# i2Nav-WHU/IC-GVINS

Measured on AMD Instinct MI355X. Metric: frames/s at 1280x720, 300 feats, 10-KF window; residual/Jacobian eval/s, higher is better.
Workload: dtype u8/int64 front-end (f32/f64 solves), f64 factors

## Files before the change

### ic-gvins_amd/csrc/image.hip

```cpp
#include <algorithm>

#include "icg_internal.h"

#define PRE_MAX_JOBS 64
struct pre_jobs {
    const uint8_t *src[PRE_MAX_JOBS];
    int32_t slot[PRE_MAX_JOBS];
    int stride;
    const int32_t *slot_ind;
};
__device__ __forceinline__ int pre_job_slot(const pre_jobs &j, int b) { return j.slot_ind ? j.slot_ind[b] : j.slot[b]; }

__global__ void k_bgr2gray(const uint8_t *bgr, int w, int h, int sstride, size_t sbatch, uint8_t *gray, int gstride,
                           size_t gbatch) {
    int x = blockIdx.x * blockDim.x + threadIdx.x;
    int y = blockIdx.y;
    int b = blockIdx.z;
    if (x >= w) return;
    const uint8_t *p = bgr + (size_t) b * sbatch + (size_t) y * sstride + 3 * x;
    gray[(size_t) b * gbatch + (size_t) y * gstride + x] =
        (uint8_t) ((p[0] * 1868 + p[1] * 9617 + p[2] * 4899 + 8192) >> 14);
}

__global__ void k_hist256(pre_jobs jobs, int w, int h, unsigned int *hist ) {
    __shared__ unsigned int sh[256];
    int b = blockIdx.y;
    sh[threadIdx.x] = 0;
    __syncthreads();
    const uint8_t *src = jobs.src[b];
    const int stride   = jobs.stride;
    int total          = src ? w * h : 0;
    for (int i = blockIdx.x * blockDim.x + threadIdx.x; i < total; i += gridDim.x * blockDim.x) {
        int y = i / w, x = i - y * w;
        atomicAdd(&sh[src[(size_t) y * stride + x]], 1u);
    }
    __syncthreads();
    if (sh[threadIdx.x]) atomicAdd(&hist[(size_t) b * 256 + threadIdx.x], sh[threadIdx.x]);
}

struct clahe_geom {
    int w, h, tw, th, clip;
    float lut_scale, inv_tw, inv_th;
};

__device__ __forceinline__ int wave_sum_i32(int v) {
    v += __builtin_amdgcn_update_dpp(0, v, 0xB1, 0xF, 0xF, false);
    v += __builtin_amdgcn_update_dpp(0, v, 0x4E, 0xF, 0xF, false);
    v += __builtin_amdgcn_update_dpp(0, v, 0x141, 0xF, 0xF, false);
    v += __builtin_amdgcn_update_dpp(0, v, 0x140, 0xF, 0xF, false);
    v += __builtin_amdgcn_update_dpp(0, v, 0x142, 0xA, 0xF, false);
    v += __builtin_amdgcn_update_dpp(0, v, 0x143, 0xC, 0xF, false);
    return __builtin_amdgcn_readlane(v, 63);
}
__device__ __forceinline__ int wave_scan_i32(int v) {
    v += __builtin_amdgcn_update_dpp(0, v, 0x111, 0xF, 0xF, true);
    v += __builtin_amdgcn_update_dpp(0, v, 0x112, 0xF, 0xF, true);
    v += __builtin_amdgcn_update_dpp(0, v, 0x114, 0xF, 0xF, true);
    v += __builtin_amdgcn_update_dpp(0, v, 0x118, 0xF, 0xF, true);
    v += __builtin_amdgcn_update_dpp(0, v, 0x142, 0xA, 0xF, false);
    v += __builtin_amdgcn_update_dpp(0, v, 0x143, 0xC, 0xF, false);
    return v;
}

__global__ __launch_bounds__(64) void k_clahe_lut(pre_jobs jobs, clahe_geom g, uint8_t *lut , int n_items) {
    __shared__ __attribute__((aligned(16))) unsigned int hist[256];
    const int lane = threadIdx.x;
    const int item = icg_xcd_chunked(blockIdx.x, n_items);
    if (item >= n_items) return;
    const int b    = item / (ICG_CLAHE_TILES * ICG_CLAHE_TILES);
    const int tile = item - b * (ICG_CLAHE_TILES * ICG_CLAHE_TILES);
    const int ty = tile / ICG_CLAHE_TILES, tx = tile - ty * ICG_CLAHE_TILES;
    const uint8_t *src = jobs.src[b];
    if (!src) return;
    const int stride   = jobs.stride;
    reinterpret_cast<uint4 *>(hist)[lane] = make_uint4(0, 0, 0, 0);
    __syncthreads();

    const int x_begin = tx * g.tw, x_end = x_begin + g.tw, y_begin = ty * g.th;
    const int xa  = x_begin & ~3;
    const int ndw = (((x_end + 3) & ~3) - xa) >> 2;
    const bool pad_small = g.th * ICG_CLAHE_TILES < 2 * g.h - 1;
    auto load_row_dword = [&](int r, int x) -> unsigned int {
        const uint8_t *row = src + (size_t) (pad_small ? icg_reflect1(y_begin + r, g.h) : icg_reflect101(y_begin + r, g.h)) * stride;
        if (x + 3 < g.w) return *reinterpret_cast<const unsigned int *>(row + x);
        unsigned int v = 0;
#pragma unroll
        for (int j = 0; j < 4; j++) v |= (unsigned int) row[icg_reflect101(x + j, g.w)] << (8 * j);
        return v;
    };
    const int nin = ndw - 2;
    const bool fast = nin >= 1 && nin <= 16 && y_begin + g.th <= g.h && xa + 4 * ndw <= g.w;
    if (fast) {
        const int d = lane & 15, q = lane >> 4;
        const bool on = d < nin;
        const uint8_t *p = src + (size_t) (y_begin + q) * stride + (xa + 4 * (on ? d + 1 : 1));
        unsigned char *hb = reinterpret_cast<unsigned char *>(hist);
        const size_t step = 4 * (size_t) stride;
        for (int r = q; r < g.th; r += 16, p += 4 * step) {
            unsigned int v[4];
            bool ok[4];
#pragma unroll
            for (int k = 0; k < 4; k++) {
                ok[k] = on && r + 4 * k < g.th;
                v[k]  = r + 4 * k < g.th ? *reinterpret_cast<const unsigned int *>(p + k * step) : 0u;
            }
#pragma unroll
            for (int k = 0; k < 4; k++) {
                if (ok[k]) {
                    atomicAdd(reinterpret_cast<unsigned int *>(hb + ((v[k] << 2) & 0x3fcu)), 1u);
                    atomicAdd(reinterpret_cast<unsigned int *>(hb + ((v[k] >> 6) & 0x3fcu)), 1u);
                    atomicAdd(reinterpret_cast<unsigned int *>(hb + ((v[k] >> 14) & 0x3fcu)), 1u);
                    atomicAdd(reinterpret_cast<unsigned int *>(hb + ((v[k] >> 22) & 0x3fcu)), 1u);
                }
            }
        }
    } else {
        {
            const int items = g.th * (nin > 0 ? nin : 0);
            const unsigned int magic = nin > 0 ? ((1u << 20) + (unsigned int) nin - 1u) / (unsigned int) nin : 0u;
            constexpr int CH = 9;
            for (int base = 0; base < items; base += 64 * CH) {
                unsigned int v[CH];
                bool ok[CH];
    #pragma unroll
                for (int k = 0; k < CH; k++) {
                    const int i = base + k * 64 + lane;
                    ok[k]       = i < items;
                    v[k]        = 0;
                    if (ok[k]) {
                        const int r = (int) (((unsigned int) i * magic) >> 20), d = 1 + i - r * nin;
                        v[k]        = load_row_dword(r, xa + 4 * d);
                    }
                }
    #pragma unroll
                for (int k = 0; k < CH; k++) {
                    if (ok[k]) {
    #pragma unroll
                        for (int j = 0; j < 4; j++) atomicAdd(&hist[(v[k] >> (8 * j)) & 0xff], 1u);
                    }
                }
            }
        }
    }
    {
        const int nedge = ndw >= 2 ? 2 : 1, items = g.th * nedge;
        for (int i = lane; i < items; i += 64) {
            const int r = nedge == 2 ? (i >> 1) : i, d = (nedge == 2 && (i & 1)) ? ndw - 1 : 0;
            const int x = xa + 4 * d;
            const unsigned int v = load_row_dword(r, x);
#pragma unroll
            for (int j = 0; j < 4; j++) {
                const int xx = x + j;
                if (xx >= x_begin && xx < x_end) atomicAdd(&hist[(v >> (8 * j)) & 0xff], 1u);
            }
        }
    }
    __syncthreads();

    const uint4 h4 = reinterpret_cast<const uint4 *>(hist)[lane];
    int hv[4]      = {(int) h4.x, (int) h4.y, (int) h4.z, (int) h4.w};
    int excess     = 0;
#pragma unroll
    for (int j = 0; j < 4; j++) {
        if (hv[j] > g.clip) {
            excess += hv[j] - g.clip;
            hv[j] = g.clip;
        }
    }
    const int clipped   = wave_sum_i32(excess);
    const int batch_add = clipped / 256;
    const int residual  = clipped - batch_add * 256;
    int step            = residual ? 256 / residual : 1;
    if (step < 1) step = 1;
    int run = 0;
#pragma unroll
    for (int j = 0; j < 4; j++) {
        const int t = 4 * lane + j;
        hv[j] += batch_add;
        if (residual != 0 && (t % step) == 0 && (t / step) < residual) hv[j]++;
        run += hv[j];
        hv[j] = run;
    }
    const int incl = wave_scan_i32(run);
    const int excl = incl - run;
    unsigned int packed = 0;
#pragma unroll
    for (int j = 0; j < 4; j++) {
        const float f = rintf((float) (excl + hv[j]) * g.lut_scale);
        int iv        = (int) f;
        iv            = iv < 0 ? 0 : (iv > 255 ? 255 : iv);
        packed |= (unsigned int) iv << (8 * j);
    }
    reinterpret_cast<unsigned int *>(lut + ((size_t) b * ICG_CLAHE_TILES * ICG_CLAHE_TILES + tile) * 256)[lane] = packed;
}

#define CLAHE_CHUNK 256
#define CLAHE_MAXCOLS 24
#define CLAHE_FCOLS 8

typedef float f32x2 __attribute__((ext_vector_type(2)));

template <bool FLT>
__device__ __forceinline__ void clahe_apply_body(const pre_jobs &jobs, const clahe_geom &g, const uint8_t *lut, uint8_t *frames, size_t slot_bytes,
                                                 int dpitch, unsigned int *slut, int strip, int chunk, int b, int t, int dslot, int p_lo, int npairs,
                                                 int x_begin) {
    const int T = ICG_CLAHE_TILES;
    int ty1 = strip - 1, ty2 = strip;
    if (ty1 < 0) ty1 = 0;
    if (ty2 > T - 1) ty2 = T - 1;
    const unsigned int *blut = reinterpret_cast<const unsigned int *>(lut + (size_t) b * T * T * 256);
    for (int i = t; i < npairs * 64; i += 256) {
        const int p = p_lo + (i >> 6), v4 = i & 63;
        int c1 = p - 1, c2 = p;
        if (c1 < 0) c1 = 0;
        if (c2 > T - 1) c2 = T - 1;
        const unsigned int A = blut[(ty1 * T + c1) * 64 + v4], B = blut[(ty1 * T + c2) * 64 + v4];
        const unsigned int C = blut[(ty2 * T + c1) * 64 + v4], D = blut[(ty2 * T + c2) * 64 + v4];
        if (FLT) {
            float4 *dst = reinterpret_cast<float4 *>(slut) + 4 * i;
#define CL_F(w, k) ((float) (((w) >> (8 * (k))) & 0xffu))
            dst[0] = make_float4(CL_F(A, 0), CL_F(B, 0), CL_F(C, 0), CL_F(D, 0));
            dst[1] = make_float4(CL_F(A, 1), CL_F(B, 1), CL_F(C, 1), CL_F(D, 1));
            dst[2] = make_float4(CL_F(A, 2), CL_F(B, 2), CL_F(C, 2), CL_F(D, 2));
            dst[3] = make_float4(CL_F(A, 3), CL_F(B, 3), CL_F(C, 3), CL_F(D, 3));
#undef CL_F
        } else {
            const unsigned int ab01 = __builtin_amdgcn_perm(B, A, 0x05010400u), ab23 = __builtin_amdgcn_perm(B, A, 0x07030602u);
            const unsigned int cd01 = __builtin_amdgcn_perm(D, C, 0x05010400u), cd23 = __builtin_amdgcn_perm(D, C, 0x07030602u);
            uint4 e;
            e.x = __builtin_amdgcn_perm(cd01, ab01, 0x05040100u);
            e.y = __builtin_amdgcn_perm(cd01, ab01, 0x07060302u);
            e.z = __builtin_amdgcn_perm(cd23, ab23, 0x05040100u);
            e.w = __builtin_amdgcn_perm(cd23, ab23, 0x07060302u);
            reinterpret_cast<uint4 *>(slut)[i] = e;
        }
    }
    __syncthreads();

    const int wave = t >> 6, lane = t & 63;
    const int x0 = x_begin + lane * 4;
    int pofs[4];
    float xa[4], xa1[4];
#pragma unroll
    for (int k = 0; k < 4; k++) {
        const int x     = x0 + k;
        const float txf = x * g.inv_tw - 0.5f;
        const int tx1   = (int) floorf(txf);
        xa[k]           = txf - tx1;
        xa1[k]          = 1.0f - xa[k];
        int p           = tx1 + 1 - p_lo;
        p               = p < 0 ? 0 : (p > npairs - 1 ? npairs - 1 : p);
        pofs[k]         = p << 8;
    }
    if (x0 >= g.w) return;

    int y_lo = (strip - 1) * g.th + g.th / 2 - 2;
    int y_hi = strip * g.th + g.th / 2 + 3;
    if (y_lo < 0) y_lo = 0;
    if (y_hi > g.h) y_hi = g.h;
    const uint8_t *src = jobs.src[b];
    const int stride   = jobs.stride;
    uint8_t *dst       = frames + (size_t) dslot * slot_bytes;
    if (FLT) {
        const float4 *sf = reinterpret_cast<const float4 *>(slut);
        for (int y = y_lo + wave; y < y_hi; y += 4) {
            const float tyf = y * g.inv_th - 0.5f;
            const int tyr   = (int) floorf(tyf);
            if (tyr != strip - 1) continue;
            const float ya = tyf - tyr, ya1 = 1.0f - ya;
            const unsigned int pin = *reinterpret_cast<const unsigned int *>(src + (size_t) y * stride + x0);
            const float4 e0 = sf[pofs[0] + (pin & 0xff)], e1 = sf[pofs[1] + ((pin >> 8) & 0xff)];
            const float4 e2 = sf[pofs[2] + ((pin >> 16) & 0xff)], e3 = sf[pofs[3] + (pin >> 24)];
            const float r0 = (e0.x * xa1[0] + e0.y * xa[0]) * ya1 + (e0.z * xa1[0] + e0.w * xa[0]) * ya;
            const float r1 = (e1.x * xa1[1] + e1.y * xa[1]) * ya1 + (e1.z * xa1[1] + e1.w * xa[1]) * ya;
            const float r2 = (e2.x * xa1[2] + e2.y * xa[2]) * ya1 + (e2.z * xa1[2] + e2.w * xa[2]) * ya;
            const float r3 = (e3.x * xa1[3] + e3.y * xa[3]) * ya1 + (e3.z * xa1[3] + e3.w * xa[3]) * ya;
            const unsigned int m0 = __float_as_uint(r0 + 12582912.f), m1 = __float_as_uint(r1 + 12582912.f);
            const unsigned int m2 = __float_as_uint(r2 + 12582912.f), m3 = __float_as_uint(r3 + 12582912.f);
            const unsigned int lo = __builtin_amdgcn_perm(m1, m0, 0x0c0c0400u), hi = __builtin_amdgcn_perm(m3, m2, 0x0c0c0400u);
            *reinterpret_cast<unsigned int *>(dst + (size_t) y * dpitch + x0) = __builtin_amdgcn_perm(hi, lo, 0x05040100u);
        }
        return;
    }
    const f32x2 XA01 = {xa[0], xa[1]}, XA23 = {xa[2], xa[3]}, XB01 = {xa1[0], xa1[1]}, XB23 = {xa1[2], xa1[3]};
    for (int y = y_lo + wave; y < y_hi; y += 4) {
        const float tyf = y * g.inv_th - 0.5f;
        const int tyr   = (int) floorf(tyf);
        if (tyr != strip - 1) continue;
        const float ya = tyf - tyr, ya1 = 1.0f - ya;
        const unsigned int pin = *reinterpret_cast<const unsigned int *>(src + (size_t) y * stride + x0);
        const unsigned int e0 = slut[pofs[0] + (pin & 0xff)], e1 = slut[pofs[1] + ((pin >> 8) & 0xff)];
        const unsigned int e2 = slut[pofs[2] + ((pin >> 16) & 0xff)], e3 = slut[pofs[3] + (pin >> 24)];
#define CL_B(e, k) ((float) (((e) >> (8 * (k))) & 0xffu))
        const f32x2 A01 = {CL_B(e0, 0), CL_B(e1, 0)}, B01 = {CL_B(e0, 1), CL_B(e1, 1)};
        const f32x2 C01 = {CL_B(e0, 2), CL_B(e1, 2)}, D01 = {CL_B(e0, 3), CL_B(e1, 3)};
        const f32x2 A23 = {CL_B(e2, 0), CL_B(e3, 0)}, B23 = {CL_B(e2, 1), CL_B(e3, 1)};
        const f32x2 C23 = {CL_B(e2, 2), CL_B(e3, 2)}, D23 = {CL_B(e2, 3), CL_B(e3, 3)};
#undef CL_B
        const f32x2 r01 = (A01 * XB01 + B01 * XA01) * ya1 + (C01 * XB01 + D01 * XA01) * ya;
        const f32x2 r23 = (A23 * XB23 + B23 * XA23) * ya1 + (C23 * XB23 + D23 * XA23) * ya;
        const float res[4] = {r01.x, r01.y, r23.x, r23.y};
        unsigned int pout = 0;
#pragma unroll
        for (int k = 0; k < 4; k++) {
            const int iv = (int) rintf(res[k]);
            pout |= (unsigned int) (iv < 0 ? 0 : (iv > 255 ? 255 : iv)) << (8 * k);
        }
        *reinterpret_cast<unsigned int *>(dst + (size_t) y * dpitch + x0) = pout;
    }
}

__global__ __launch_bounds__(256) void k_clahe_apply(pre_jobs jobs, clahe_geom g, const uint8_t *lut, uint8_t *frames,
                                                     size_t slot_bytes, int dpitch) {
    __shared__ __attribute__((aligned(16))) unsigned int slut[CLAHE_FCOLS * 256 * 4];
    static_assert(CLAHE_FCOLS * 4 >= CLAHE_MAXCOLS, "the byte form must fit the same array");
    const int strip = blockIdx.x;
    const int chunk = blockIdx.y;
    const int b     = blockIdx.z;
    const int t     = threadIdx.x;
    const int dslot = pre_job_slot(jobs, b);
    if (!jobs.src[b] || dslot < 0) return;
    const int x_begin = chunk * CLAHE_CHUNK;
    int x_end         = x_begin + CLAHE_CHUNK;
    if (x_end > g.w) x_end = g.w;
    const int p_lo   = (int) floorf(x_begin * g.inv_tw - 0.5f) + 1;
    const int p_hi   = (int) floorf((x_end - 1) * g.inv_tw - 0.5f) + 1;
    const int npairs = p_hi - p_lo + 1;
    if (npairs <= CLAHE_FCOLS)
        clahe_apply_body<true>(jobs, g, lut, frames, slot_bytes, dpitch, slut, strip, chunk, b, t, dslot, p_lo, npairs, x_begin);
    else
        clahe_apply_body<false>(jobs, g, lut, frames, slot_bytes, dpitch, slut, strip, chunk, b, t, dslot, p_lo, npairs, x_begin);
}

#define PR_STRIP_OUT 128
struct pr_sel {
    unsigned int a, b, t, v;
};
typedef unsigned int pr_u3 __attribute__((ext_vector_type(3)));
__device__ __forceinline__ pr_u3 pr_load(const uint8_t *row, unsigned int wx) {
    typedef pr_u3 __attribute__((aligned(4))) u3a;
    return *reinterpret_cast<const u3a *>(row + wx);
}
template <bool EDGE> __device__ __forceinline__ unsigned int pr_hsum(const pr_u3 E, const pr_sel &S) {
    unsigned int A, B, V4;
    if (EDGE) {
        A  = __builtin_amdgcn_perm(E.y, E.x, S.a);
        B  = __builtin_amdgcn_perm(E.y, E.x, S.b);
        V4 = __builtin_amdgcn_perm(E.z, __builtin_amdgcn_perm(E.y, E.x, S.t), S.v);
    } else {
        A  = __builtin_amdgcn_alignbyte(E.y, E.x, 2);
        B  = E.y;
        V4 = E.z & 0xffu;
    }
    const unsigned int h0 = __builtin_amdgcn_udot4(B, 0x00010000u, __builtin_amdgcn_udot4(A, 0x04060401u, 0u, false), false);
    const unsigned int h1 = __builtin_amdgcn_udot4(B, 0x04060401u, V4, false);
    return h0 | (h1 << 16);
}

template <bool EDGE>
__device__ __forceinline__ void pr_band(const uint8_t *src, int sh, int spitch, uint8_t *dst, int dpitch, int i0, int i1, unsigned int wx,
                                        const pr_sel &S, unsigned int dcol, bool store) {
    auto srow = [&](int r) { return src + (unsigned int) __builtin_amdgcn_readfirstlane(icg_reflect1(r, sh) * spitch); };
    unsigned int hA = pr_hsum<EDGE>(pr_load(srow(2 * i0 - 2), wx), S), hB = pr_hsum<EDGE>(pr_load(srow(2 * i0 - 1), wx), S);
    unsigned int hC = pr_hsum<EDGE>(pr_load(srow(2 * i0), wx), S);
// ... 38 lines not shown
        S.t = 0x0c0c0c00u | (unsigned int) (ix[6] & 7);
        S.v = ix[6] >= 8 ? (0x0c0c0c04u + (unsigned int) (ix[6] - 8)) : 0x0c0c0c00u;
    }
    const int i0 = band * band_rows, i1 = min(i0 + band_rows, dh);
    if (i0 >= i1) return;
    const uint8_t *src = slot + src_off;
    uint8_t *dst       = slot + dst_off;
    const bool store   = oj < dw;
    if (edge)
        pr_band<true>(src, sh, spitch, dst, dpitch, i0, i1, (unsigned int) wx, S, (unsigned int) oj, store);
    else
        pr_band<false>(src, sh, spitch, dst, dpitch, i0, i1, (unsigned int) wx, S, (unsigned int) oj, store);
}

__global__ void k_hist_mean(int n, const unsigned int *hist, int w, int h, double *mean) {
    const int k = blockIdx.x * blockDim.x + threadIdx.x;
    if (k >= n) return;
    double acc = 0;
    for (int i = 0; i < 256; i++) {
        const float hf = (float) hist[(size_t) k * 256 + i];
        acc += hf * (float) i / 256.0;
    }
    mean[k] = acc / ((double) w * h);
}

static int preprocess_impl(icg_ctx *ctx, int n, const int32_t *slots, const int32_t *d_slot_ind, const uint8_t *const *images, int stride, int channels,
                           int src_on_device, double *hist_mean, double *d_hist_mean) {
    if (!ctx || n < 0 || (n > 0 && ((!slots && !d_slot_ind) || !images))) return ICG_ERR_INVALID;
    if (n == 0) return ICG_OK;
    if (n > ctx->cfg.max_batch) return icg_fail(ctx, ICG_ERR_CAPACITY, "preprocess batch %d > max_batch %d", n, ctx->cfg.max_batch);
    if (channels != 1 && channels != 3) return icg_fail(ctx, ICG_ERR_INVALID, "channels must be 1 or 3");
    const int w = ctx->cfg.width, h = ctx->cfg.height;
    if (stride < w * channels) return icg_fail(ctx, ICG_ERR_INVALID, "stride too small");
    for (int k = 0; k < n && slots; k++)
        if (slots[k] < 0 || slots[k] >= ctx->cfg.n_slots || !images[k]) return icg_fail(ctx, ICG_ERR_INVALID, "bad slot/image %d", k);
    ICG_HIP(ctx, hipSetDevice(ctx->cfg.device));
    const bool want_hist = hist_mean || d_hist_mean;

    const int T = ICG_CLAHE_TILES;
    int ew = w, eh = h;
    if (w % T != 0 || h % T != 0) {
        ew = w + (T - w % T);
        eh = h + (T - h % T);
    }
    clahe_geom g;
    g.w = w;
    g.h = h;
    g.tw = ew / T;
    g.th = eh / T;
    int area    = g.tw * g.th;
    g.lut_scale = 255.0f / area;
    g.clip      = (int) (3.0 * area / 256);
    if (g.clip < 1) g.clip = 1;
    g.inv_tw = 1.0f / g.tw;
    g.inv_th = 1.0f / g.th;
    static_assert(ICG_CLAHE_TILES + 1 <= CLAHE_MAXCOLS, "k_clahe_apply's staged LUT must hold every interpolation column pair");

    const size_t raw_batch = (size_t) ctx->raw_pitch * h;
    hipMemcpyKind kind     = src_on_device ? hipMemcpyDeviceToDevice : hipMemcpyHostToDevice;
    unsigned int *d_hist   = nullptr;
    if (want_hist) {
        if (int rcd = icg_arena_drain(ctx)) return rcd;
        ctx->arena_off = 0;
        int rc         = icg_arena_reserve(ctx, sizeof(unsigned int) * 256 * (size_t) n + 4096);
        if (rc) return rc;
        d_hist = icg_d<unsigned int>(ctx, icg_arena_alloc(ctx, sizeof(unsigned int) * 256 * (size_t) n));
// ... 23 lines not shown
            bool direct = src_on_device && (stride % 4 == 0);
            for (int k = 0; k < m && direct; k++) direct = (((uintptr_t) images[base + k]) % 4) == 0;
            if (direct) {
                for (int k = 0; k < m; k++) jobs.src[k] = images[base + k];
                jobs.stride = stride;
            } else {
                const bool linear = stride == w && ctx->raw_pitch == w;
                for (int k = 0; k < m; k++) {
                    uint8_t *dst = ctx->d_raw + (size_t) (base + k) * raw_batch;
                    if (!images[base + k]) {
                        jobs.src[k] = nullptr;
                        continue;
                    }
                    if (linear)
                        ICG_HIP(ctx, hipMemcpyAsync(dst, images[base + k], (size_t) w * h, kind, ctx->stream));
                    else
                        ICG_HIP(ctx, hipMemcpy2DAsync(dst, ctx->raw_pitch, images[base + k], stride, w, h, kind, ctx->stream));
                    jobs.src[k] = dst;
                }
                jobs.stride = ctx->raw_pitch;
            }
        }
        if (want_hist) {
            icg_prof_scope ps(ctx, "hist256");
            hipLaunchKernelGGL(k_hist256, dim3(64, m), dim3(256), 0, ctx->stream, jobs, w, h, d_hist + (size_t) base * 256);
        }
        uint8_t *lut = ctx->d_lut + (size_t) base * T * T * 256;
        {
            icg_prof_scope ps(ctx, "clahe_lut");
            hipLaunchKernelGGL(k_clahe_lut, dim3(icg_xcd_grid(T * T * m)), dim3(64), 0, ctx->stream, jobs, g, lut, T * T * m);
        }
        {
            icg_prof_scope ps(ctx, "clahe_apply");
            hipLaunchKernelGGL(k_clahe_apply, dim3(T + 1, (w + CLAHE_CHUNK - 1) / CLAHE_CHUNK, m), dim3(256), 0, ctx->stream, jobs,
                               g, lut, ctx->d_frames, ctx->slot_bytes, ctx->lv[0].pitch);
        }
        for (int l = 1; l < ctx->n_levels; l++) {
            icg_prof_scope ps(ctx, "pyrdown_rows");
            const icg_level &a = ctx->lv[l - 1], &bb = ctx->lv[l];
            const int n_strips = (bb.w + PR_STRIP_OUT - 1) / PR_STRIP_OUT;
            const int band_rows = bb.h >= 256 ? 32 : bb.h >= 128 ? 16 : 8;
            const int n_bands   = (bb.h + band_rows - 1) / band_rows;
            const int n_tasks   = n_strips * n_bands * m;
            hipLaunchKernelGGL(k_pyrdown_rows, dim3(icg_xcd_grid(n_tasks)), dim3(64), 0, ctx->stream, ctx->d_frames, ctx->slot_bytes, jobs,
                               (unsigned int) a.off, a.w, a.h, a.pitch, (unsigned int) bb.off, bb.w, bb.h, bb.pitch, n_strips, n_bands, band_rows,
                               n_tasks);
        }
    }
    if (d_hist_mean) hipLaunchKernelGGL(k_hist_mean, dim3((n + 63) / 64), dim3(64), 0, ctx->stream, n, d_hist, w, h, d_hist_mean);
    ICG_HIP(ctx, hipGetLastError());
    if (d_hist_mean) ctx->arena_off = 0;
    if (!hist_mean) return ICG_OK;

    std::vector<unsigned int> hc((size_t) n * 256);
    ICG_HIP(ctx, hipMemcpyAsync(hc.data(), d_hist, sizeof(unsigned int) * 256 * (size_t) n, hipMemcpyDeviceToHost, ctx->stream));
    ICG_HIP(ctx, hipStreamSynchronize(ctx->stream));
    icg_prof_collect(ctx);
    for (int k = 0; k < n; k++) {
        double acc = 0;
        for (int i = 0; i < 256; i++) {
            float hf = (float) hc[(size_t) k * 256 + i];
            acc += hf * (float) i / 256.0;
        }
        hist_mean[k] = acc / ((double) w * h);
    }
    ctx->arena_off = 0;
    return ICG_OK;
// ... 24 lines not shown
```

Baseline: 162,800.

## Unify CLAHE histogram into templated row sweep and restructure LUT apply loop

Replaces the fast/slow/edge histogram paths in the CLAHE LUT kernel with a single templated sweep. Edge dwords are masked by redirecting out-of-tile bytes to per-lane dummy bins, and 24-bit unsigned row offsets replace size_t arithmetic. The clip-redistribution step uses a constant step table and shared-memory flags instead of per-bin divisions and modulos. The float interpolation apply loop ballots the active rows once per 64-row chunk, so waves no longer test each row individually. It also raises PRE_MAX_JOBS and adds a size check on the source plane so the 32-bit offsets stay valid.

```diff
diff --git a/ic-gvins_amd/csrc/image.hip b/ic-gvins_amd/csrc/image.hip
--- a/ic-gvins_amd/csrc/image.hip
+++ b/ic-gvins_amd/csrc/image.hip
@@ -2,7 +2,9 @@
 
 #include "icg_internal.h"
 
-#define PRE_MAX_JOBS 64
+#ifndef PRE_MAX_JOBS
+#define PRE_MAX_JOBS 192
+#endif
 struct pre_jobs {
     const uint8_t *src[PRE_MAX_JOBS];
     int32_t slot[PRE_MAX_JOBS];
@@ -62,8 +64,59 @@
     return v;
 }
 
+struct clahe_step_table {
+    int v[256];
+    constexpr clahe_step_table() : v() {
+        v[0] = 1;
+        for (int r = 1; r < 256; r++) v[r] = 256 / r;
+    }
+};
+__constant__ clahe_step_table c_clahe_step = clahe_step_table();
+
+template <int U, bool BYTES, bool BOTTOM, bool CHECK>
+__device__ __forceinline__ void clahe_hist_rows(const uint8_t *src, unsigned char *hb, const unsigned int (&am)[4], const unsigned int (&ov)[4],
+                                                const unsigned int (&xo)[4], int y0, int rs, int y_end, int h, unsigned int stride) {
+    unsigned int v[U];
+    bool ok[U];
+    const unsigned int ro0 = BOTTOM ? 0u : __umul24((unsigned int) y0, stride), rstep = (unsigned int) rs * stride;
+#pragma unroll
+    for (int k = 0; k < U; k++) {
+        const int y = y0 + k * rs;
+        ok[k] = !CHECK || y < y_end;
+        v[k]  = 0;
+        if (ok[k]) {
+            const unsigned int ro = BOTTOM ? __umul24((unsigned int) icg_reflect1(y, h), stride) : ro0 + (unsigned int) k * rstep;
+            if (BYTES) {
+                v[k] = (unsigned int) src[ro + xo[0]] | ((unsigned int) src[ro + xo[1]] << 8) | ((unsigned int) src[ro + xo[2]] << 16) |
+                       ((unsigned int) src[ro + xo[3]] << 24);
+            } else {
+                v[k] = *reinterpret_cast<const unsigned int *>(src + (ro + xo[0]));
+            }
+        }
+    }
+#pragma unroll
+    for (int k = 0; k < U; k++) {
+        if (ok[k]) {
+            atomicAdd(reinterpret_cast<unsigned int *>(hb + (((v[k] << 2) & am[0]) | ov[0])), 1u);
+            atomicAdd(reinterpret_cast<unsigned int *>(hb + (((v[k] >> 6) & am[1]) | ov[1])), 1u);
+            atomicAdd(reinterpret_cast<unsigned int *>(hb + (((v[k] >> 14) & am[2]) | ov[2])), 1u);
+            atomicAdd(reinterpret_cast<unsigned int *>(hb + (((v[k] >> 22) & am[3]) | ov[3])), 1u);
+        }
+    }
+}
+
+template <bool BYTES, bool BOTTOM>
+__device__ __forceinline__ void clahe_hist_sweep(const uint8_t *src, unsigned char *hb, const unsigned int (&am)[4], const unsigned int (&ov)[4],
+                                                 const unsigned int (&xo)[4], int y_begin, int q, int lgrs, int th, int h, unsigned int stride) {
+    const int rs = 1 << lgrs, full = th >> lgrs, y_end = y_begin + th;
+    int s = 0;
+    for (; s + 4 <= full; s += 4) clahe_hist_rows<4, BYTES, BOTTOM, false>(src, hb, am, ov, xo, y_begin + q + s * rs, rs, y_end, h, stride);
+    for (; s < full; s++) clahe_hist_rows<1, BYTES, BOTTOM, false>(src, hb, am, ov, xo, y_begin + q + s * rs, rs, y_end, h, stride);
+    if (th & (rs - 1)) clahe_hist_rows<1, BYTES, BOTTOM, true>(src, hb, am, ov, xo, y_begin + q + s * rs, rs, y_end, h, stride);
+}
+
 __global__ __launch_bounds__(64) void k_clahe_lut(pre_jobs jobs, clahe_geom g, uint8_t *lut , int n_items) {
-    __shared__ __attribute__((aligned(16))) unsigned int hist[256];
+    __shared__ __attribute__((aligned(16))) unsigned int hist[256 + 64];
     const int lane = threadIdx.x;
     const int item = icg_xcd_chunked(blockIdx.x, n_items);
     if (item >= n_items) return;
@@ -72,88 +125,40 @@
     const int ty = tile / ICG_CLAHE_TILES, tx = tile - ty * ICG_CLAHE_TILES;
     const uint8_t *src = jobs.src[b];
     if (!src) return;
-    const int stride   = jobs.stride;
+    const unsigned int stride = (unsigned int) jobs.stride;
     reinterpret_cast<uint4 *>(hist)[lane] = make_uint4(0, 0, 0, 0);
     __syncthreads();
 
     const int x_begin = tx * g.tw, x_end = x_begin + g.tw, y_begin = ty * g.th;
     const int xa  = x_begin & ~3;
     const int ndw = (((x_end + 3) & ~3) - xa) >> 2;
-    const bool pad_small = g.th * ICG_CLAHE_TILES < 2 * g.h - 1;
-    auto load_row_dword = [&](int r, int x) -> unsigned int {
-        const uint8_t *row = src + (size_t) (pad_small ? icg_reflect1(y_begin + r, g.h) : icg_reflect101(y_begin + r, g.h)) * stride;
-        if (x + 3 < g.w) return *reinterpret_cast<const unsigned int *>(row + x);
-        unsigned int v = 0;
-#pragma unroll
-        for (int j = 0; j < 4; j++) v |= (unsigned int) row[icg_reflect101(x + j, g.w)] << (8 * j);
-        return v;
-    };
-    const int nin = ndw - 2;
-    const bool fast = nin >= 1 && nin <= 16 && y_begin + g.th <= g.h && xa + 4 * ndw <= g.w;
-    if (fast) {
-        const int d = lane & 15, q = lane >> 4;
-        const bool on = d < nin;
-        const uint8_t *p = src + (size_t) (y_begin + q) * stride + (xa + 4 * (on ? d + 1 : 1));
-        unsigned char *hb = reinterpret_cast<unsigned char *>(hist);
-        const size_t step = 4 * (size_t) stride;
-        for (int r = q; r < g.th; r += 16, p += 4 * step) {
-            unsigned int v[4];
-            bool ok[4];
-#pragma unroll
-            for (int k = 0; k < 4; k++) {
-                ok[k] = on && r + 4 * k < g.th;
-                v[k]  = r + 4 * k < g.th ? *reinterpret_cast<const unsigned int *>(p + k * step) : 0u;
-            }
-#pragma unroll
-            for (int k = 0; k < 4; k++) {
-                if (ok[k]) {
-                    atomicAdd(reinterpret_cast<unsigned int *>(hb + ((v[k] << 2) & 0x3fcu)), 1u);
-                    atomicAdd(reinterpret_cast<unsigned int *>(hb + ((v[k] >> 6) & 0x3fcu)), 1u);
-                    atomicAdd(reinterpret_cast<unsigned int *>(hb + ((v[k] >> 14) & 0x3fcu)), 1u);
-                    atomicAdd(reinterpret_cast<unsigned int *>(hb + ((v[k] >> 22) & 0x3fcu)), 1u);
-                }
-            }
-        }
-    } else {
-        {
-            const int items = g.th * (nin > 0 ? nin : 0);
-            const unsigned int magic = nin > 0 ? ((1u << 20) + (unsigned int) nin - 1u) / (unsigned int) nin : 0u;
-            constexpr int CH = 9;
-            for (int base = 0; base < items; base += 64 * CH) {
-                unsigned int v[CH];
-                bool ok[CH];
-    #pragma unroll
-                for (int k = 0; k < CH; k++) {
-                    const int i = base + k * 64 + lane;
-                    ok[k]       = i < items;
-                    v[k]        = 0;
-                    if (ok[k]) {
-                        const int r = (int) (((unsigned int) i * magic) >> 20), d = 1 + i - r * nin;
-                        v[k]        = load_row_dword(r, xa + 4 * d);
-                    }
-                }
-    #pragma unroll
-                for (int k = 0; k < CH; k++) {
-                    if (ok[k]) {
-    #pragma unroll
-                        for (int j = 0; j < 4; j++) atomicAdd(&hist[(v[k] >> (8 * j)) & 0xff], 1u);
-                    }
-                }
-            }
-        }
-    }
-    {
-        const int nedge = ndw >= 2 ? 2 : 1, items = g.th * nedge;
-        for (int i = lane; i < items; i += 64) {
-            const int r = nedge == 2 ? (i >> 1) : i, d = (nedge == 2 && (i & 1)) ? ndw - 1 : 0;
-            const int x = xa + 4 * d;
-            const unsigned int v = load_row_dword(r, x);
-#pragma unroll
-            for (int j = 0; j < 4; j++) {
-                const int xx = x + j;
-                if (xx >= x_begin && xx < x_end) atomicAdd(&hist[(v >> (8 * j)) & 0xff], 1u);
-            }
-        }
+    int lg = 0;
+    while ((1 << lg) < ndw && lg < 6) lg++;
+    const int G = 1 << lg, q = lane >> lg;
+    const bool bottom = y_begin + g.th > g.h;
+    const bool bytes  = xa + 4 * ndw > g.w;
+    unsigned char *hb = reinterpret_cast<unsigned char *>(hist);
+    for (int c0 = 0; c0 < ndw; c0 += G) {
+        const int d = c0 + (lane & (G - 1));
+        const bool on = d < ndw;
+        const int xd = xa + 4 * (on ? d : ndw - 1);
+        unsigned int am[4], ov[4], xo[4];
+#pragma unroll
+        for (int j = 0; j < 4; j++) {
+            const int xx   = xd + j;
+            const bool use = on && xx >= x_begin && xx < x_end;
+            am[j] = use ? 0x3fcu : 0u;
+            ov[j] = use ? 0u : 1024u + 4u * (unsigned int) lane;
+            xo[j] = (unsigned int) (bytes ? icg_reflect1(xx, g.w) : xx);
+        }
+        if (bytes && bottom)
+            clahe_hist_sweep<true, true>(src, hb, am, ov, xo, y_begin, q, 6 - lg, g.th, g.h, stride);
+        else if (bytes)
+            clahe_hist_sweep<true, false>(src, hb, am, ov, xo, y_begin, q, 6 - lg, g.th, g.h, stride);
+        else if (bottom)
+            clahe_hist_sweep<false, true>(src, hb, am, ov, xo, y_begin, q, 6 - lg, g.th, g.h, stride);
+        else
+            clahe_hist_sweep<false, false>(src, hb, am, ov, xo, y_begin, q, 6 - lg, g.th, g.h, stride);
     }
     __syncthreads();
 
@@ -168,16 +173,25 @@
         }
     }
     const int clipped   = wave_sum_i32(excess);
-    const int batch_add = clipped / 256;
-    const int residual  = clipped - batch_add * 256;
-    int step            = residual ? 256 / residual : 1;
-    if (step < 1) step = 1;
+    const int batch_add = clipped >> 8;
+    const int residual  = clipped & 255;
+    unsigned int flags = 0;
+    if (residual != 0) {
+        const int step = c_clahe_step.v[residual];
+        __syncthreads();
+        hist[lane] = 0;
+        __syncthreads();
+        for (int k = lane; k < residual; k += 64) {
+            const unsigned int bin = __umul24((unsigned int) k, (unsigned int) step);
+            if (bin < 256u) hb[bin] = 1;
+        }
+        __syncthreads();
+        flags = hist[lane];
+    }
     int run = 0;
 #pragma unroll
     for (int j = 0; j < 4; j++) {
-        const int t = 4 * lane + j;
-        hv[j] += batch_add;
-        if (residual != 0 && (t % step) == 0 && (t / step) < residual) hv[j]++;
+        hv[j] += batch_add + (int) ((flags >> (8 * j)) & 1u);
         run += hv[j];
         hv[j] = run;
     }
@@ -237,7 +251,7 @@
     }
     __syncthreads();
 
-    const int wave = t >> 6, lane = t & 63;
+    const int wave = __builtin_amdgcn_readfirstlane(t >> 6), lane = t & 63;
     const int x0 = x_begin + lane * 4;
     int pofs[4];
     float xa[4], xa1[4];
@@ -252,7 +266,6 @@
         p               = p < 0 ? 0 : (p > npairs - 1 ? npairs - 1 : p);
         pofs[k]         = p << 8;
     }
-    if (x0 >= g.w) return;
 
     int y_lo = (strip - 1) * g.th + g.th / 2 - 2;
     int y_hi = strip * g.th + g.th / 2 + 3;
@@ -263,25 +276,38 @@
     uint8_t *dst       = frames + (size_t) dslot * slot_bytes;
     if (FLT) {
         const float4 *sf = reinterpret_cast<const float4 *>(slut);
-        for (int y = y_lo + wave; y < y_hi; y += 4) {
-            const float tyf = y * g.inv_th - 0.5f;
+        const bool act   = x0 < g.w;
+        const unsigned int xl = (unsigned int) (act ? x0 : x_begin);
+        for (int c0 = y_lo; c0 < y_hi; c0 += 64) {
+            const int yc    = c0 + lane;
+            const float tyf = yc * g.inv_th - 0.5f;
             const int tyr   = (int) floorf(tyf);
-            if (tyr != strip - 1) continue;
-            const float ya = tyf - tyr, ya1 = 1.0f - ya;
-            const unsigned int pin = *reinterpret_cast<const unsigned int *>(src + (size_t) y * stride + x0);
-            const float4 e0 = sf[pofs[0] + (pin & 0xff)], e1 = sf[pofs[1] + ((pin >> 8) & 0xff)];
-            const float4 e2 = sf[pofs[2] + ((pin >> 16) & 0xff)], e3 = sf[pofs[3] + (pin >> 24)];
-            const float r0 = (e0.x * xa1[0] + e0.y * xa[0]) * ya1 + (e0.z * xa1[0] + e0.w * xa[0]) * ya;
-            const float r1 = (e1.x * xa1[1] + e1.y * xa[1]) * ya1 + (e1.z * xa1[1] + e1.w * xa[1]) * ya;
-            const float r2 = (e2.x * xa1[2] + e2.y * xa[2]) * ya1 + (e2.z * xa1[2] + e2.w * xa[2]) * ya;
-            const float r3 = (e3.x * xa1[3] + e3.y * xa[3]) * ya1 + (e3.z * xa1[3] + e3.w * xa[3]) * ya;
-            const unsigned int m0 = __float_as_uint(r0 + 12582912.f), m1 = __float_as_uint(r1 + 12582912.f);
-            const unsigned int m2 = __float_as_uint(r2 + 12582912.f), m3 = __float_as_uint(r3 + 12582912.f);
-            const unsigned int lo = __builtin_amdgcn_perm(m1, m0, 0x0c0c0400u), hi = __builtin_amdgcn_perm(m3, m2, 0x0c0c0400u);
-            *reinterpret_cast<unsigned int *>(dst + (size_t) y * dpitch + x0) = __builtin_amdgcn_perm(hi, lo, 0x05040100u);
+            const float ya_l = tyf - tyr, ya1_l = 1.0f - ya_l;
+            const unsigned long long rows = __builtin_amdgcn_ballot_w64(yc < y_hi && tyr == strip - 1);
+            if (rows != 0) {
+                const int first = (int) __builtin_ctzll(rows), end = first + (int) __builtin_popcountll(rows);
+                for (int i = first + wave; i < end; i += 4) {
+                    const float ya  = __int_as_float(__builtin_amdgcn_readlane(__float_as_int(ya_l), i));
+                    const float ya1 = __int_as_float(__builtin_amdgcn_readlane(__float_as_int(ya1_l), i));
+                    const uint8_t *srow = src + (size_t) (c0 + i) * stride;
+                    uint8_t *drow       = dst + (size_t) (c0 + i) * dpitch;
+                    const unsigned int pin = *reinterpret_cast<const unsigned int *>(srow + xl);
+                    const float4 e0 = sf[pofs[0] + (pin & 0xff)], e1 = sf[pofs[1] + ((pin >> 8) & 0xff)];
+                    const float4 e2 = sf[pofs[2] + ((pin >> 16) & 0xff)], e3 = sf[pofs[3] + (pin >> 24)];
+                    const float r0 = (e0.x * xa1[0] + e0.y * xa[0]) * ya1 + (e0.z * xa1[0] + e0.w * xa[0]) * ya;
+                    const float r1 = (e1.x * xa1[1] + e1.y * xa[1]) * ya1 + (e1.z * xa1[1] + e1.w * xa[1]) * ya;
+                    const float r2 = (e2.x * xa1[2] + e2.y * xa[2]) * ya1 + (e2.z * xa1[2] + e2.w * xa[2]) * ya;
+                    const float r3 = (e3.x * xa1[3] + e3.y * xa[3]) * ya1 + (e3.z * xa1[3] + e3.w * xa[3]) * ya;
+                    const unsigned int m0 = __float_as_uint(r0 + 12582912.f), m1 = __float_as_uint(r1 + 12582912.f);
+                    const unsigned int m2 = __float_as_uint(r2 + 12582912.f), m3 = __float_as_uint(r3 + 12582912.f);
+                    const unsigned int lo = __builtin_amdgcn_perm(m1, m0, 0x0c0c0400u), hi = __builtin_amdgcn_perm(m3, m2, 0x0c0c0400u);
+                    if (act) *reinterpret_cast<unsigned int *>(drow + xl) = __builtin_amdgcn_perm(hi, lo, 0x05040100u);
+                }
+            }
         }
         return;
     }
+    if (x0 >= g.w) return;
     const f32x2 XA01 = {xa[0], xa[1]}, XA23 = {xa[2], xa[3]}, XB01 = {xa1[0], xa1[1]}, XB23 = {xa1[2], xa1[3]};
     for (int y = y_lo + wave; y < y_hi; y += 4) {
         const float tyf = y * g.inv_th - 0.5f;
@@ -434,6 +460,8 @@
     if (channels != 1 && channels != 3) return icg_fail(ctx, ICG_ERR_INVALID, "channels must be 1 or 3");
     const int w = ctx->cfg.width, h = ctx->cfg.height;
     if (stride < w * channels) return icg_fail(ctx, ICG_ERR_INVALID, "stride too small");
+    if ((uint64_t) stride * (uint64_t) h > 0xffffffffull || stride >= (1 << 24) || h >= (1 << 24))
+        return icg_fail(ctx, ICG_ERR_INVALID, "source plane of %d x %d bytes is too large", stride, h);
     for (int k = 0; k < n && slots; k++)
         if (slots[k] < 0 || slots[k] >= ctx->cfg.n_slots || !images[k]) return icg_fail(ctx, ICG_ERR_INVALID, "bad slot/image %d", k);
     ICG_HIP(ctx, hipSetDevice(ctx->cfg.device));
```

New measurement: 162,100. No clear change (-0.5%).

## Band CLAHE apply over multiple strips per block and ballot-select rows

Applied to the files above, without the earlier changes.

The CLAHE apply kernel now has each block loop over a band of four tile strips instead of one, rebuilding the shared interpolation LUT per strip. Rows belonging to each strip are found with a wave ballot, which avoids per-row floor tests and skipped iterations. The LUT kernel's clip-redistribution step replaces integer division and modulo with a constexpr table of step and reciprocal values plus 24-bit multiplies. Fewer blocks cut launch and scheduling overhead, but parallelism drops and extra __syncthreads barriers are added between strips.

```diff
diff --git a/ic-gvins_amd/csrc/image.hip b/ic-gvins_amd/csrc/image.hip
--- a/ic-gvins_amd/csrc/image.hip
+++ b/ic-gvins_amd/csrc/image.hip
@@ -61,6 +61,19 @@
     v += __builtin_amdgcn_update_dpp(0, v, 0x143, 0xC, 0xF, false);
     return v;
 }
+
+struct clahe_step_table {
+    unsigned int v[256];
+};
+static constexpr clahe_step_table clahe_make_step_table() {
+    clahe_step_table t{};
+    for (unsigned int r = 0; r < 256; r++) {
+        const unsigned int step = r ? (256u / r ? 256u / r : 1u) : 1u;
+        t.v[r]                  = ((65536u + step - 1u) / step) << 9 | step;
+    }
+    return t;
+}
+__constant__ clahe_step_table CLAHE_STEP = clahe_make_step_table();
 
 __global__ __launch_bounds__(64) void k_clahe_lut(pre_jobs jobs, clahe_geom g, uint8_t *lut , int n_items) {
     __shared__ __attribute__((aligned(16))) unsigned int hist[256];
@@ -167,17 +180,18 @@
             hv[j] = g.clip;
         }
     }
-    const int clipped   = wave_sum_i32(excess);
-    const int batch_add = clipped / 256;
-    const int residual  = clipped - batch_add * 256;
-    int step            = residual ? 256 / residual : 1;
-    if (step < 1) step = 1;
+    const int clipped      = wave_sum_i32(excess);
+    const int batch_add    = clipped >> 8;
+    const int residual     = clipped & 255;
+    const unsigned int sm  = CLAHE_STEP.v[residual];
+    const unsigned int step = sm & 511u, magic = sm >> 9;
     int run = 0;
 #pragma unroll
     for (int j = 0; j < 4; j++) {
-        const int t = 4 * lane + j;
-        hv[j] += batch_add;
-        if (residual != 0 && (t % step) == 0 && (t / step) < residual) hv[j]++;
+        const unsigned int t = 4u * (unsigned int) lane + j;
+        const unsigned int q = __umul24(t, magic) >> 16;
+        const unsigned int d = t - __umul24(q, step);
+        hv[j] += batch_add + ((((d << 8) | q) < (unsigned int) residual) ? 1 : 0);
         run += hv[j];
         hv[j] = run;
     }
@@ -197,47 +211,16 @@
 #define CLAHE_CHUNK 256
 #define CLAHE_MAXCOLS 24
 #define CLAHE_FCOLS 8
+#define CLAHE_BAND 4
 
 typedef float f32x2 __attribute__((ext_vector_type(2)));
 
 template <bool FLT>
 __device__ __forceinline__ void clahe_apply_body(const pre_jobs &jobs, const clahe_geom &g, const uint8_t *lut, uint8_t *frames, size_t slot_bytes,
-                                                 int dpitch, unsigned int *slut, int strip, int chunk, int b, int t, int dslot, int p_lo, int npairs,
-                                                 int x_begin) {
+                                                 int dpitch, unsigned int *slut, int strip_lo, int strip_hi, int b, int t, int dslot, int p_lo,
+                                                 int npairs, int x_begin) {
     const int T = ICG_CLAHE_TILES;
-    int ty1 = strip - 1, ty2 = strip;
-    if (ty1 < 0) ty1 = 0;
-    if (ty2 > T - 1) ty2 = T - 1;
-    const unsigned int *blut = reinterpret_cast<const unsigned int *>(lut + (size_t) b * T * T * 256);
-    for (int i = t; i < npairs * 64; i += 256) {
-        const int p = p_lo + (i >> 6), v4 = i & 63;
-        int c1 = p - 1, c2 = p;
-        if (c1 < 0) c1 = 0;
-        if (c2 > T - 1) c2 = T - 1;
-        const unsigned int A = blut[(ty1 * T + c1) * 64 + v4], B = blut[(ty1 * T + c2) * 64 + v4];
-        const unsigned int C = blut[(ty2 * T + c1) * 64 + v4], D = blut[(ty2 * T + c2) * 64 + v4];
-        if (FLT) {
-            float4 *dst = reinterpret_cast<float4 *>(slut) + 4 * i;
-#define CL_F(w, k) ((float) (((w) >> (8 * (k))) & 0xffu))
-            dst[0] = make_float4(CL_F(A, 0), CL_F(B, 0), CL_F(C, 0), CL_F(D, 0));
-            dst[1] = make_float4(CL_F(A, 1), CL_F(B, 1), CL_F(C, 1), CL_F(D, 1));
-            dst[2] = make_float4(CL_F(A, 2), CL_F(B, 2), CL_F(C, 2), CL_F(D, 2));
-            dst[3] = make_float4(CL_F(A, 3), CL_F(B, 3), CL_F(C, 3), CL_F(D, 3));
-#undef CL_F
-        } else {
-            const unsigned int ab01 = __builtin_amdgcn_perm(B, A, 0x05010400u), ab23 = __builtin_amdgcn_perm(B, A, 0x07030602u);
-            const unsigned int cd01 = __builtin_amdgcn_perm(D, C, 0x05010400u), cd23 = __builtin_amdgcn_perm(D, C, 0x07030602u);
-            uint4 e;
-            e.x = __builtin_amdgcn_perm(cd01, ab01, 0x05040100u);
-            e.y = __builtin_amdgcn_perm(cd01, ab01, 0x07060302u);
-            e.z = __builtin_amdgcn_perm(cd23, ab23, 0x05040100u);
-            e.w = __builtin_amdgcn_perm(cd23, ab23, 0x07060302u);
-            reinterpret_cast<uint4 *>(slut)[i] = e;
-        }
-    }
-    __syncthreads();
-
-    const int wave = t >> 6, lane = t & 63;
+    const int wave = __builtin_amdgcn_readfirstlane(t >> 6), lane = t & 63;
     const int x0 = x_begin + lane * 4;
     int pofs[4];
     float xa[4], xa1[4];
@@ -252,61 +235,102 @@
         p               = p < 0 ? 0 : (p > npairs - 1 ? npairs - 1 : p);
         pofs[k]         = p << 8;
     }
-    if (x0 >= g.w) return;
-
-    int y_lo = (strip - 1) * g.th + g.th / 2 - 2;
-    int y_hi = strip * g.th + g.th / 2 + 3;
-    if (y_lo < 0) y_lo = 0;
-    if (y_hi > g.h) y_hi = g.h;
+    const bool live = x0 < g.w;
+    const f32x2 XA01 = {xa[0], xa[1]}, XA23 = {xa[2], xa[3]}, XB01 = {xa1[0], xa1[1]}, XB23 = {xa1[2], xa1[3]};
     const uint8_t *src = jobs.src[b];
     const int stride   = jobs.stride;
     uint8_t *dst       = frames + (size_t) dslot * slot_bytes;
-    if (FLT) {
-        const float4 *sf = reinterpret_cast<const float4 *>(slut);
-        for (int y = y_lo + wave; y < y_hi; y += 4) {
-            const float tyf = y * g.inv_th - 0.5f;
-            const int tyr   = (int) floorf(tyf);
-            if (tyr != strip - 1) continue;
-            const float ya = tyf - tyr, ya1 = 1.0f - ya;
-            const unsigned int pin = *reinterpret_cast<const unsigned int *>(src + (size_t) y * stride + x0);
-            const float4 e0 = sf[pofs[0] + (pin & 0xff)], e1 = sf[pofs[1] + ((pin >> 8) & 0xff)];
-            const float4 e2 = sf[pofs[2] + ((pin >> 16) & 0xff)], e3 = sf[pofs[3] + (pin >> 24)];
-            const float r0 = (e0.x * xa1[0] + e0.y * xa[0]) * ya1 + (e0.z * xa1[0] + e0.w * xa[0]) * ya;
-            const float r1 = (e1.x * xa1[1] + e1.y * xa[1]) * ya1 + (e1.z * xa1[1] + e1.w * xa[1]) * ya;
-            const float r2 = (e2.x * xa1[2] + e2.y * xa[2]) * ya1 + (e2.z * xa1[2] + e2.w * xa[2]) * ya;
-            const float r3 = (e3.x * xa1[3] + e3.y * xa[3]) * ya1 + (e3.z * xa1[3] + e3.w * xa[3]) * ya;
-            const unsigned int m0 = __float_as_uint(r0 + 12582912.f), m1 = __float_as_uint(r1 + 12582912.f);
-            const unsigned int m2 = __float_as_uint(r2 + 12582912.f), m3 = __float_as_uint(r3 + 12582912.f);
-            const unsigned int lo = __builtin_amdgcn_perm(m1, m0, 0x0c0c0400u), hi = __builtin_amdgcn_perm(m3, m2, 0x0c0c0400u);
-            *reinterpret_cast<unsigned int *>(dst + (size_t) y * dpitch + x0) = __builtin_amdgcn_perm(hi, lo, 0x05040100u);
-        }
-        return;
-    }
-    const f32x2 XA01 = {xa[0], xa[1]}, XA23 = {xa[2], xa[3]}, XB01 = {xa1[0], xa1[1]}, XB23 = {xa1[2], xa1[3]};
-    for (int y = y_lo + wave; y < y_hi; y += 4) {
-        const float tyf = y * g.inv_th - 0.5f;
-        const int tyr   = (int) floorf(tyf);
-        if (tyr != strip - 1) continue;
-        const float ya = tyf - tyr, ya1 = 1.0f - ya;
-        const unsigned int pin = *reinterpret_cast<const unsigned int *>(src + (size_t) y * stride + x0);
-        const unsigned int e0 = slut[pofs[0] + (pin & 0xff)], e1 = slut[pofs[1] + ((pin >> 8) & 0xff)];
-        const unsigned int e2 = slut[pofs[2] + ((pin >> 16) & 0xff)], e3 = slut[pofs[3] + (pin >> 24)];
+    const unsigned int xo    = (unsigned int) (live ? x0 : x_begin);
+    const unsigned int *blut = reinterpret_cast<const unsigned int *>(lut + (size_t) b * T * T * 256);
+    const float4 *sf         = reinterpret_cast<const float4 *>(slut);
+
+    for (int strip = strip_lo; strip < strip_hi; strip++) {
+        int ty1 = strip - 1, ty2 = strip;
+        if (ty1 < 0) ty1 = 0;
+        if (ty2 > T - 1) ty2 = T - 1;
+        if (strip != strip_lo) __syncthreads();
+        for (int i = t; i < npairs * 64; i += 256) {
+            const int p = p_lo + (i >> 6), v4 = i & 63;
+            int c1 = p - 1, c2 = p;
+            if (c1 < 0) c1 = 0;
+            if (c2 > T - 1) c2 = T - 1;
+            const unsigned int A = blut[(ty1 * T + c1) * 64 + v4], B = blut[(ty1 * T + c2) * 64 + v4];
+            const unsigned int C = blut[(ty2 * T + c1) * 64 + v4], D = blut[(ty2 * T + c2) * 64 + v4];
+            if (FLT) {
+                float4 *e = reinterpret_cast<float4 *>(slut) + 4 * i;
+#define CL_F(w, k) ((float) (((w) >> (8 * (k))) & 0xffu))
+                e[0] = make_float4(CL_F(A, 0), CL_F(B, 0), CL_F(C, 0), CL_F(D, 0));
+                e[1] = make_float4(CL_F(A, 1), CL_F(B, 1), CL_F(C, 1), CL_F(D, 1));
+                e[2] = make_float4(CL_F(A, 2), CL_F(B, 2), CL_F(C, 2), CL_F(D, 2));
+                e[3] = make_float4(CL_F(A, 3), CL_F(B, 3), CL_F(C, 3), CL_F(D, 3));
+#undef CL_F
+            } else {
+                const unsigned int ab01 = __builtin_amdgcn_perm(B, A, 0x05010400u), ab23 = __builtin_amdgcn_perm(B, A, 0x07030602u);
+                const unsigned int cd01 = __builtin_amdgcn_perm(D, C, 0x05010400u), cd23 = __builtin_amdgcn_perm(D, C, 0x07030602u);
+                uint4 e;
+                e.x = __builtin_amdgcn_perm(cd01, ab01, 0x05040100u);
+                e.y = __builtin_amdgcn_perm(cd01, ab01, 0x07060302u);
+                e.z = __builtin_amdgcn_perm(cd23, ab23, 0x05040100u);
+                e.w = __builtin_amdgcn_perm(cd23, ab23, 0x07060302u);
+                reinterpret_cast<uint4 *>(slut)[i] = e;
+            }
+        }
+        __syncthreads();
+
+        int y_lo = (strip - 1) * g.th + g.th / 2 - 2;
+        int y_hi = strip * g.th + g.th / 2 + 3;
+        if (y_lo < 0) y_lo = 0;
+        if (y_hi > g.h) y_hi = g.h;
+        for (int base = y_lo; base < y_hi; base += 64) {
+            const int yc      = base + lane;
+            const float tyf   = yc * g.inv_th - 0.5f;
+            const int tyr     = (int) floorf(tyf);
+            const float ya_c  = tyf - tyr;
+            const float ya1_c = 1.0f - ya_c;
+            const unsigned long long rows = __builtin_amdgcn_ballot_w64(tyr == strip - 1 && yc < y_hi);
+            {
+                const int n = y_hi - base < 64 ? y_hi - base : 64;
+                for (int r = wave; r < n; r += 4) {
+                    if (!((rows >> r) & 1ull)) continue;
+                    const float ya  = __int_as_float(__builtin_amdgcn_readlane(__float_as_int(ya_c), r));
+                    const float ya1 = __int_as_float(__builtin_amdgcn_readlane(__float_as_int(ya1_c), r));
+                    const int y     = base + r;
+                    const unsigned int pin = *reinterpret_cast<const unsigned int *>(src + ((unsigned int) (y * stride) + xo));
+                    unsigned int *out      = reinterpret_cast<unsigned int *>(dst + ((unsigned int) (y * dpitch) + xo));
+                    if (FLT) {
+                        const float4 e0 = sf[pofs[0] + (pin & 0xff)], e1 = sf[pofs[1] + ((pin >> 8) & 0xff)];
+                        const float4 e2 = sf[pofs[2] + ((pin >> 16) & 0xff)], e3 = sf[pofs[3] + (pin >> 24)];
+                        const float r0 = (e0.x * xa1[0] + e0.y * xa[0]) * ya1 + (e0.z * xa1[0] + e0.w * xa[0]) * ya;
+                        const float r1 = (e1.x * xa1[1] + e1.y * xa[1]) * ya1 + (e1.z * xa1[1] + e1.w * xa[1]) * ya;
+                        const float r2 = (e2.x * xa1[2] + e2.y * xa[2]) * ya1 + (e2.z * xa1[2] + e2.w * xa[2]) * ya;
+                        const float r3 = (e3.x * xa1[3] + e3.y * xa[3]) * ya1 + (e3.z * xa1[3] + e3.w * xa[3]) * ya;
+                        const unsigned int m0 = __float_as_uint(r0 + 12582912.f), m1 = __float_as_uint(r1 + 12582912.f);
+                        const unsigned int m2 = __float_as_uint(r2 + 12582912.f), m3 = __float_as_uint(r3 + 12582912.f);
+                        const unsigned int lo = __builtin_amdgcn_perm(m1, m0, 0x0c0c0400u), hi = __builtin_amdgcn_perm(m3, m2, 0x0c0c0400u);
+                        if (live) *out = __builtin_amdgcn_perm(hi, lo, 0x05040100u);
+                    } else {
+                        const unsigned int e0 = slut[pofs[0] + (pin & 0xff)], e1 = slut[pofs[1] + ((pin >> 8) & 0xff)];
+                        const unsigned int e2 = slut[pofs[2] + ((pin >> 16) & 0xff)], e3 = slut[pofs[3] + (pin >> 24)];
 #define CL_B(e, k) ((float) (((e) >> (8 * (k))) & 0xffu))
-        const f32x2 A01 = {CL_B(e0, 0), CL_B(e1, 0)}, B01 = {CL_B(e0, 1), CL_B(e1, 1)};
-        const f32x2 C01 = {CL_B(e0, 2), CL_B(e1, 2)}, D01 = {CL_B(e0, 3), CL_B(e1, 3)};
-        const f32x2 A23 = {CL_B(e2, 0), CL_B(e3, 0)}, B23 = {CL_B(e2, 1), CL_B(e3, 1)};
-        const f32x2 C23 = {CL_B(e2, 2), CL_B(e3, 2)}, D23 = {CL_B(e2, 3), CL_B(e3, 3)};
+                        const f32x2 A01 = {CL_B(e0, 0), CL_B(e1, 0)}, B01 = {CL_B(e0, 1), CL_B(e1, 1)};
+                        const f32x2 C01 = {CL_B(e0, 2), CL_B(e1, 2)}, D01 = {CL_B(e0, 3), CL_B(e1, 3)};
+                        const f32x2 A23 = {CL_B(e2, 0), CL_B(e3, 0)}, B23 = {CL_B(e2, 1), CL_B(e3, 1)};
+                        const f32x2 C23 = {CL_B(e2, 2), CL_B(e3, 2)}, D23 = {CL_B(e2, 3), CL_B(e3, 3)};
 #undef CL_B
-        const f32x2 r01 = (A01 * XB01 + B01 * XA01) * ya1 + (C01 * XB01 + D01 * XA01) * ya;
-        const f32x2 r23 = (A23 * XB23 + B23 * XA23) * ya1 + (C23 * XB23 + D23 * XA23) * ya;
-        const float res[4] = {r01.x, r01.y, r23.x, r23.y};
-        unsigned int pout = 0;
-#pragma unroll
-        for (int k = 0; k < 4; k++) {
-            const int iv = (int) rintf(res[k]);
-            pout |= (unsigned int) (iv < 0 ? 0 : (iv > 255 ? 255 : iv)) << (8 * k);
-        }
-        *reinterpret_cast<unsigned int *>(dst + (size_t) y * dpitch + x0) = pout;
+                        const f32x2 r01 = (A01 * XB01 + B01 * XA01) * ya1 + (C01 * XB01 + D01 * XA01) * ya;
+                        const f32x2 r23 = (A23 * XB23 + B23 * XA23) * ya1 + (C23 * XB23 + D23 * XA23) * ya;
+                        const float res[4] = {r01.x, r01.y, r23.x, r23.y};
+                        unsigned int pout = 0;
+#pragma unroll
+                        for (int k = 0; k < 4; k++) {
+                            const int iv = (int) rintf(res[k]);
+                            pout |= (unsigned int) (iv < 0 ? 0 : (iv > 255 ? 255 : iv)) << (8 * k);
+                        }
+                        if (live) *out = pout;
+                    }
+                }
+            }
+        }
     }
 }
 
@@ -314,11 +338,12 @@
                                                      size_t slot_bytes, int dpitch) {
     __shared__ __attribute__((aligned(16))) unsigned int slut[CLAHE_FCOLS * 256 * 4];
     static_assert(CLAHE_FCOLS * 4 >= CLAHE_MAXCOLS, "the byte form must fit the same array");
-    const int strip = blockIdx.x;
-    const int chunk = blockIdx.y;
-    const int b     = blockIdx.z;
-    const int t     = threadIdx.x;
-    const int dslot = pre_job_slot(jobs, b);
+    const int strip_lo = blockIdx.x * CLAHE_BAND;
+    const int strip_hi = strip_lo + CLAHE_BAND < ICG_CLAHE_TILES + 1 ? strip_lo + CLAHE_BAND : ICG_CLAHE_TILES + 1;
+    const int chunk    = blockIdx.y;
+    const int b        = blockIdx.z;
+    const int t        = threadIdx.x;
+    const int dslot    = __builtin_amdgcn_readfirstlane(pre_job_slot(jobs, b));
     if (!jobs.src[b] || dslot < 0) return;
     const int x_begin = chunk * CLAHE_CHUNK;
     int x_end         = x_begin + CLAHE_CHUNK;
@@ -327,9 +352,9 @@
     const int p_hi   = (int) floorf((x_end - 1) * g.inv_tw - 0.5f) + 1;
     const int npairs = p_hi - p_lo + 1;
     if (npairs <= CLAHE_FCOLS)
-        clahe_apply_body<true>(jobs, g, lut, frames, slot_bytes, dpitch, slut, strip, chunk, b, t, dslot, p_lo, npairs, x_begin);
+        clahe_apply_body<true>(jobs, g, lut, frames, slot_bytes, dpitch, slut, strip_lo, strip_hi, b, t, dslot, p_lo, npairs, x_begin);
     else
-        clahe_apply_body<false>(jobs, g, lut, frames, slot_bytes, dpitch, slut, strip, chunk, b, t, dslot, p_lo, npairs, x_begin);
+        clahe_apply_body<false>(jobs, g, lut, frames, slot_bytes, dpitch, slut, strip_lo, strip_hi, b, t, dslot, p_lo, npairs, x_begin);
 }
 
 #define PR_STRIP_OUT 128
@@ -523,7 +548,7 @@
         }
         {
             icg_prof_scope ps(ctx, "clahe_apply");
-            hipLaunchKernelGGL(k_clahe_apply, dim3(T + 1, (w + CLAHE_CHUNK - 1) / CLAHE_CHUNK, m), dim3(256), 0, ctx->stream, jobs,
+            hipLaunchKernelGGL(k_clahe_apply, dim3((T + 1 + CLAHE_BAND - 1) / CLAHE_BAND, (w + CLAHE_CHUNK - 1) / CLAHE_CHUNK, m), dim3(256), 0, ctx->stream, jobs,
                                g, lut, ctx->d_frames, ctx->slot_bytes, ctx->lv[0].pitch);
         }
         for (int l = 1; l < ctx->n_levels; l++) {
```

Result: no change. 161,900 before, 162,200 after, median of 2 (+0.2%).
